# benjisu03/grayshift

Measured on AMD Instinct MI355X. Metric: Msamples/sec (primary+secondary rays), higher is better.
Workload: dtype f64; 1 GPU; C4: bouncing_spheres_50 1920x1080, 512 spp; tile=64, parallelism=tiles1, tile_plan=round-robin, collective=none, launch=one process, 1 device(s): gs_multi_create once, gs_multi_render per frame, seed=1, rays_per_frame=2921120250

## Files before the change

### __graft_entry__.py

```python
import os
import sys

ROOT = os.path.dirname(os.path.abspath(__file__))


def build():
    sys.path.insert(0, ROOT)
    from grayshift_amd import build as b
    b.build_product()
    b.build_oracle()
    b.build_kat()
    import grayshift_amd
    from grayshift_amd import _native


def smoke():
    sys.path.insert(0, ROOT)
    sys.path.insert(0, os.path.join(ROOT, "oracle"))
    import numpy as np
    import grayshift_amd as g
    from grayshift_amd import scenes
    import oracle

    sc = scenes.config("C4", width=48, spp=4)
    out, gc = g.render(sc, seed=7)
    ref, rc = oracle.render(sc, seed=7)
    d = float(np.abs(out.astype(np.float64) - ref.astype(np.float64)).max())
    if not (d < 1e-3) or gc != rc:
        raise AssertionError("smoke parity failed: max|d|=%g counters gpu=%s oracle=%s" % (d, gc, rc))
    print("smoke ok: C4 48x27x4spp max|d|=%g rays=%d" % (d, gc["rays"]))


if __name__ == "__main__":
    build()
# ... 3 lines not shown
```

### bindings/grayshift_gpu.rs

```rust
#![allow(non_camel_case_types)]

use std::os::raw::{c_char, c_void};

pub type gs_status = i32;
pub const GS_OK: gs_status = 0;
pub const GS_ERR_ARG: gs_status = -1;
pub const GS_ERR_HIP: gs_status = -2;
pub const GS_ERR_OOM: gs_status = -3;
pub const GS_ERR_UNSUPPORTED: gs_status = -4;
pub const GS_ERR_NO_DEVICE: gs_status = -5;

pub const GS_REF_SHIFT: u32 = 28;
pub const GS_REF_NONE: u32 = 0;
pub const GS_REF_NODE: u32 = 1;
pub const GS_REF_SPHERE: u32 = 2;
pub const GS_REF_MSPHERE: u32 = 3;
pub const GS_REF_QUAD: u32 = 4;
pub const GS_REF_TRIANGLE: u32 = 5;
pub const GS_REF_LIST: u32 = 6;
pub const GS_REF_INSTANCE: u32 = 7;
pub const GS_REF_MEDIUM: u32 = 8;
pub const GS_REF_BUILD_MEMBER: u32 = 15;
pub const GS_ABI_VERSION: i32 = 11;
pub const fn gs_make_ref(kind: u32, idx: u32) -> u32 { (kind << GS_REF_SHIFT) | (idx & 0x0FFF_FFFF) }
// ... 137 lines not shown
    pub feat: i32, pub node_steps: i32, pub cert_boxes: i32, pub nodes_per_leaf: f64, pub other_leaf_frac: f64,
    pub placement: i32, pub long_samples: i32, pub pilot_ms: f64,
}

#[repr(C)] #[derive(Clone, Copy)]
pub struct gs_debug_leaf_stage {
    pub tquads: *const c_void, pub n_quads: u32, pub n_cubes: u32, pub lds_quads: u32, pub lds_cubes: u32,
}

#[link(name = "grayshift")]
extern "C" {
    pub fn gs_last_error() -> *const c_char;
    pub fn gs_version() -> i32;
    pub fn gs_set_tuning(shade_batch: i32, blocks_per_cu: i32, leaf_batch: i32, sample_chunk: i32) -> gs_status;
    pub fn gs_debug_set_partial_budget(bytes: u64) -> gs_status;
    pub fn gs_debug_set_guided_tail(fine_chunk: i32, tail_pct: i32) -> gs_status;
    pub fn gs_set_node_steps(node_steps: i32) -> gs_status;
    pub fn gs_set_camera_batch(cam_batch: i32) -> gs_status;
    pub fn gs_set_placement(mode: i32) -> gs_status;
    pub fn gs_set_adaptive_mode(mode: i32) -> gs_status;
    pub fn gs_debug_set_round_items(mode: i32) -> gs_status;
    pub fn gs_debug_set_cube_lists(on: i32) -> gs_status;
    pub fn gs_debug_set_cert_boxes(on: i32) -> gs_status;
    pub fn gs_debug_set_mirror_budget(bytes: i64) -> gs_status;
    pub fn gs_debug_record_visits(scene: *const gs_device_scene, cam: *const gs_camera, ss: *const gs_sample_settings,
                                  seed: u64, part: *const gs_partition, d_packed_rgb: *mut f32, d_visits: *mut u32,
                                  stream: *mut c_void) -> gs_status;
    pub fn gs_debug_last_launch_feat(scene: *const gs_device_scene, feat: *mut i32) -> gs_status;
    pub fn gs_debug_device_scene_record(scene: *const gs_device_scene, out: *mut c_void, out_bytes: i64) -> gs_status;
    pub fn gs_debug_leaf_stage_record(scene: *const gs_device_scene, out: *mut gs_debug_leaf_stage, out_bytes: i64) -> gs_status;
    pub fn gs_device_scene_create(scene: *const gs_flat_scene, out: *mut *mut gs_device_scene) -> gs_status;
    pub fn gs_device_scene_destroy(scene: *mut gs_device_scene) -> gs_status;
    pub fn gs_device_scene_info(scene: *const gs_device_scene, out: *mut gs_scene_info) -> gs_status;
    pub fn gs_partition_capacity(cam: *const gs_camera, part: *const gs_partition) -> i64;
    pub fn gs_render_tiles_async(scene: *const gs_device_scene, cam: *const gs_camera, ss: *const gs_sample_settings,
                                 seed: u64, part: *const gs_partition, d_packed_rgb: *mut f32,
                                 d_counters: *mut gs_counters, stream: *mut c_void) -> gs_status;
    pub fn gs_render_tiles_debug_async(scene: *const gs_device_scene, cam: *const gs_camera,
                                       ss: *const gs_sample_settings, seed: u64, part: *const gs_partition,
                                       d_packed_rgb: *mut f32, d_counters: *mut gs_counters,
                                       d_item_visits: *mut u32, stream: *mut c_void) -> gs_status;
    pub fn gs_unpack_tiles_async(cam: *const gs_camera, world_size: i32, tile_w: i32, tile_h: i32, capacity: i64,
                                 d_gathered: *const f32, d_frame: *mut f32, stream: *mut c_void) -> gs_status;
    pub fn gs_render_tiles_ex_async(scene: *const gs_device_scene, cam: *const gs_camera,
                                    ss: *const gs_sample_settings, seed: u64, part: *const gs_partition,
                                    out: *const gs_render_outputs, d_counters: *mut gs_counters,
// ... 331 lines not shown
```

### grayshift_amd/_native.py

```python
import ctypes as C
import os

HERE = os.path.dirname(os.path.abspath(__file__))
LIB_PATH = os.environ.get("GS_LIB") or os.path.join(HERE, "libgrayshift.so")

GS_OBJ_SPHERE, GS_OBJ_MOVING_SPHERE, GS_OBJ_QUAD, GS_OBJ_TRIANGLE = 1, 2, 3, 4
GS_OBJ_LIST, GS_OBJ_BVH, GS_OBJ_TRANSLATE, GS_OBJ_ROTATE_Y, GS_OBJ_CUBE, GS_OBJ_MEDIUM = 5, 6, 7, 8, 9, 10
GS_MAT_LAMBERTIAN, GS_MAT_METAL, GS_MAT_DIELECTRIC, GS_MAT_DIFFUSE_LIGHT, GS_MAT_ISOTROPIC = 1, 2, 3, 4, 5
GS_TEX_SOLID, GS_TEX_CHECKERED, GS_TEX_IMAGE, GS_TEX_NOISE = 1, 2, 3, 4
GS_BG_SOLID, GS_BG_HDRI = 1, 2
GS_ABI_VERSION = 11
GS_OK, GS_ERR_ARG, GS_ERR_HIP, GS_ERR_OOM, GS_ERR_UNSUPPORTED, GS_ERR_NO_DEVICE = 0, -1, -2, -3, -4, -5

D3 = C.c_double * 3


class gs_object(C.Structure):
    _fields_ = [("kind", C.c_int32), ("material", C.c_int32), ("first", C.c_int32), ("count", C.c_int32),
                ("p", C.c_double * 9)]


class gs_material_spec(C.Structure):
    _fields_ = [("kind", C.c_int32), ("texture", C.c_int32), ("p", C.c_double * 4)]

# ... 222 lines not shown
        d["counters"] = self.counters.as_dict()
        return d


class gs_debug_leaf_stage(C.Structure):
    _fields_ = [("tquads", C.c_void_p), ("n_quads", C.c_uint32), ("n_cubes", C.c_uint32), ("lds_quads", C.c_uint32),
                ("lds_cubes", C.c_uint32)]


_P = C.c_void_p
SIGNATURES = {
    "gs_last_error": (C.c_char_p, []),
    "gs_version": (C.c_int32, []),
    "gs_set_tuning": (C.c_int32, [C.c_int32, C.c_int32, C.c_int32, C.c_int32]),
    "gs_debug_set_partial_budget": (C.c_int32, [C.c_uint64]),
    "gs_debug_set_guided_tail": (C.c_int32, [C.c_int32, C.c_int32]),
    "gs_set_node_steps": (C.c_int32, [C.c_int32]),
    "gs_set_camera_batch": (C.c_int32, [C.c_int32]),
    "gs_set_placement": (C.c_int32, [C.c_int32]),
    "gs_set_adaptive_mode": (C.c_int32, [C.c_int32]),
    "gs_debug_set_round_items": (C.c_int32, [C.c_int32]),
    "gs_debug_set_cube_lists": (C.c_int32, [C.c_int32]),
    "gs_debug_set_cert_boxes": (C.c_int32, [C.c_int32]),
    "gs_debug_set_mirror_budget": (C.c_int32, [C.c_int64]),
    "gs_debug_record_visits": (C.c_int32, [_P, C.POINTER(gs_camera), C.POINTER(gs_sample_settings), C.c_uint64,
                                           C.POINTER(gs_partition), _P, _P, _P]),
    "gs_debug_last_launch_feat": (C.c_int32, [_P, C.POINTER(C.c_int32)]),
    "gs_debug_device_scene_record": (C.c_int32, [_P, _P, C.c_int64]),
    "gs_debug_leaf_stage_record": (C.c_int32, [_P, C.POINTER(gs_debug_leaf_stage), C.c_int64]),
    "gs_device_scene_create": (C.c_int32, [_P, C.POINTER(_P)]),
    "gs_device_scene_destroy": (C.c_int32, [_P]),
    "gs_device_scene_info": (C.c_int32, [_P, C.POINTER(gs_scene_info)]),
    "gs_partition_capacity": (C.c_int64, [C.POINTER(gs_camera), C.POINTER(gs_partition)]),
    "gs_render_tiles_async": (C.c_int32, [_P, C.POINTER(gs_camera), C.POINTER(gs_sample_settings), C.c_uint64,
                                          C.POINTER(gs_partition), _P, _P, _P]),
    "gs_render_tiles_debug_async": (C.c_int32, [_P, C.POINTER(gs_camera), C.POINTER(gs_sample_settings), C.c_uint64,
                                                C.POINTER(gs_partition), _P, _P, _P, _P]),
    "gs_unpack_tiles_async": (C.c_int32, [C.POINTER(gs_camera), C.c_int32, C.c_int32, C.c_int32, C.c_int64, _P, _P,
                                          _P]),
    "gs_render_tiles_ex_async": (C.c_int32, [_P, C.POINTER(gs_camera), C.POINTER(gs_sample_settings), C.c_uint64,
                                             C.POINTER(gs_partition), C.POINTER(gs_render_outputs), _P, _P]),
    "gs_unpack_tiles_u8_async": (C.c_int32, [C.POINTER(gs_camera), C.c_int32, C.c_int32, C.c_int32, C.c_int64, _P,
                                             _P, _P]),
    "gs_ppm_max_bytes": (C.c_int64, [C.c_int32, C.c_int32]),
    "gs_ppm_scratch_bytes": (C.c_int64, [C.c_int32, C.c_int32]),
    "gs_ppm_encode_async": (C.c_int32, [_P, C.c_int32, C.c_int32, _P, C.c_int64, _P, _P, C.c_int64, _P]),
# ... 143 lines not shown
```

### grayshift_amd/build.py

```python
import argparse
import glob
import os
import subprocess
import sys

HERE = os.path.dirname(os.path.abspath(__file__))
ROOT = os.path.dirname(HERE)
LIB = os.path.join(HERE, "libgrayshift.so")
ORACLE_DIR = os.path.join(ROOT, "oracle")
ORACLE_LIB = os.path.join(ORACLE_DIR, "liboracle.so")

SOURCES = [
    os.path.join(HERE, "csrc", "device", "render.hip"),
    os.path.join(HERE, "csrc", "device", "output.hip"),
    os.path.join(HERE, "csrc", "device", "bvh_build.hip"),
    os.path.join(HERE, "csrc", "host", "scene.cpp"),
    os.path.join(HERE, "csrc", "host", "launch.cpp"),
    os.path.join(HERE, "csrc", "host", "world.cpp"),
    os.path.join(HERE, "csrc", "host", "camera.cpp"),
    os.path.join(HERE, "csrc", "host", "host_capi.cpp"),
    os.path.join(HERE, "csrc", "host", "multi_gpu.cpp"),
]


# ... 45 lines not shown
    if verbose:
        print(" ".join(cmd), flush=True)
    subprocess.run(cmd, check=True)
    os.replace(tmp, lib)
    return lib


KAT_SRC = os.path.join(ROOT, "tests", "hip", "kat_device.hip")
KAT_LIB = os.path.join(ROOT, "tests", "hip", "libkat_device.so")


def build_kat(force=False, verbose=False):
    deps = [KAT_SRC] + _headers()
    if not force and not _stale(KAT_LIB, deps):
        return KAT_LIB
    cmd = [HIPCC] + COMMON + ["-x", "hip", "--offload-arch=" + ARCH, "-shared", "-o", KAT_LIB + ".tmp", KAT_SRC]
    if verbose:
        print(" ".join(cmd), flush=True)
    subprocess.run(cmd, check=True)
    os.replace(KAT_LIB + ".tmp", KAT_LIB)
    return KAT_LIB


def build_oracle(force=False, verbose=False):
    if force and os.path.exists(ORACLE_LIB):
        os.remove(ORACLE_LIB)
    subprocess.run(["make", "-s", "-C", ORACLE_DIR], check=True,
                   stdout=None if verbose else subprocess.DEVNULL)
    return ORACLE_LIB


def main(argv=None):
    ap = argparse.ArgumentParser()
    ap.add_argument("--force", action="store_true")
    ap.add_argument("--no-oracle", action="store_true")
    ap.add_argument("-v", "--verbose", action="store_true")
    ap.add_argument("--variant", action="append", metavar="NAME:FLAGS", default=[],
                    help="also build variants/NAME.so with extra FLAGS (A/B), e.g. --variant 'v4:-DGS_MIN_WAVES=4'")
    ap.add_argument("--resource-usage", action="store_true",
                    help="print per-kernel VGPR/SGPR/LDS/occupancy (hipcc remarks)")
    a = ap.parse_args(argv)
    extra = ["-Rpass-analysis=kernel-resource-usage"] if a.resource_usage else []
    import concurrent.futures as cf

    def variant(spec):
        name, _, flags = spec.partition(":")
        path = os.path.join(HERE, "variants", name + ".so")
        os.makedirs(os.path.dirname(path), exist_ok=True)
        build_product(force=True, verbose=a.verbose, extra=extra + flags.split(), out=path)
        return "variant %s %s" % (path, flags)

    with cf.ThreadPoolExecutor(max_workers=4) as ex:
        jobs = [ex.submit(build_product, force=a.force or a.resource_usage, verbose=a.verbose, extra=extra)]
        jobs += [ex.submit(variant, spec) for spec in a.variant]
        for j in jobs[1:]:
            print(j.result())
        jobs[0].result()
    if not a.no_oracle:
        build_oracle(force=a.force, verbose=a.verbose)
        build_kat(force=a.force, verbose=a.verbose)
    print("built", LIB, "" if a.no_oracle else ORACLE_LIB)


if __name__ == "__main__":
    sys.exit(main())
```

### grayshift_amd/csrc/device/geometry.hpp

```cpp
#pragma once
#include "../../../include/grayshift_gpu.h"
#include "kernel_abi.hpp"
#include "devmath.hpp"

namespace gsd {

struct Ray {
    d3 o, d;
    double time;
};

__device__ __forceinline__ DNode load_node(const DNode* p) {
    const uint4* q = reinterpret_cast<const uint4*>(p);
    const uint4 a = q[0], b = q[1], c = q[2], d = q[3];
    DNode n;
    n.mnx = __hiloint2double((int)a.y, (int)a.x);
    n.mny = __hiloint2double((int)a.w, (int)a.z);
    n.mnz = __hiloint2double((int)b.y, (int)b.x);
    n.mxx = __hiloint2double((int)b.w, (int)b.z);
    n.mxy = __hiloint2double((int)c.y, (int)c.x);
    n.mxz = __hiloint2double((int)c.w, (int)c.z);
    n.left = d.x;
    n.right = d.y;
    n.pad0 = d.z;
// ... 109 lines not shown
    return c;
}
__device__ __forceinline__ bool box_cert_dt(float mnx, float mny, float mnz, float mxx, float mxy, float mxz,
                                            const RayCert& c, float tmin32, float closest32, float& d, float& thr) {
    const gs_f2 t0 = __builtin_elementwise_fma(gs_f2{mnx, mny}, c.ixy, c.oxy);
    const gs_f2 t1 = __builtin_elementwise_fma(gs_f2{mxx, mxy}, c.ixy, c.oxy);
    const gs_f2 tz = __builtin_elementwise_fma(gs_f2{mnz, mxz}, c.izz, c.ozz);
    const float t0x = t0.x, t1x = t1.x, t0y = t0.y, t1y = t1.y, t0z = tz.x, t1z = tz.y;
    const float lo = __builtin_fmaxf(__builtin_fmaxf(tmin32, __builtin_fminf(t0x, t1x)),
                                     __builtin_fmaxf(__builtin_fminf(t0y, t1y), __builtin_fminf(t0z, t1z)));
    const float hi = __builtin_fminf(__builtin_fminf(closest32, __builtin_fmaxf(t0x, t1x)),
                                     __builtin_fminf(__builtin_fmaxf(t0y, t1y), __builtin_fmaxf(t0z, t1z)));
    d = hi - lo;
    thr = __builtin_fmaf(GS_CERT_K, hi + lo, c.r2);
    return d > thr;
}
__device__ __forceinline__ bool box_cert(float mnx, float mny, float mnz, float mxx, float mxy, float mxz,
                                         const RayCert& c, float tmin32, float closest32, bool& undecided) {
    float d, thr;
    const bool h = box_cert_dt(mnx, mny, mnz, mxx, mxy, mxz, c, tmin32, closest32, d, thr);
    undecided = !h && d >= -thr;
    return h;
}
__device__ __forceinline__ DNode box64(const TBox& b) {
    DNode n;
    n.mnx = b.mnx;
    n.mny = b.mny;
    n.mnz = b.mnz;
    n.mxx = b.mxx;
    n.mxy = b.mxy;
    n.mxz = b.mxz;
    n.left = n.right = n.pad0 = n.pad1 = 0;
    return n;
}

__device__ __forceinline__ bool sphere_accept_rr(d3 c, double rr, const Ray& ray, double a, double tmin, double tmax,
                                            double& t_out) {
    d3 oc = sub(c, ray.o);
    double h = dot(ray.d, oc);
    double cc = len2(oc) - rr;
    double disc = h * h - a * cc;
    t_out = tmax;
    if (disc < 0.0) return false;
    double sq = sqrt(disc);
    double t = (h - sq) / a;
    if (!(tmin < t && t < tmax)) {
// ... 157 lines not shown
```

### grayshift_amd/csrc/device/kernel_abi.hpp

```cpp
#pragma once
#include <hip/hip_runtime_api.h>
#include <stddef.h>
#include <stdint.h>

#include "../../../include/grayshift_gpu.h"

#ifndef GS_BLOCK
#define GS_BLOCK 1024
#endif
#ifndef GS_MIN_WAVES
#define GS_MIN_WAVES 4
#endif
#define GS_MAX_CHAIN 16
#ifndef GS_ROUND_WHOLE_MAX_BATCH
#define GS_ROUND_WHOLE_MAX_BATCH 256
#endif
#define GS_NESTED_STACK 32
#define GS_FEAT_MEDIA 1
#define GS_FEAT_NESTED 2
#define GS_FEAT_LEAFRUN 4
#define GS_FEAT_LDSTREE 8
#define GS_FEAT_MIXED 16
#define GS_FEAT_VISITS 32
#define GS_FEAT_SPHLEAF 64
// ... 178 lines not shown
struct ViewBatch {
    gs_view v[GS_VIEW_BATCH];
    uint32_t first, n;
};
static_assert(sizeof(gs_view) % 8 == 0 && sizeof(ViewBatch) <= 3072, "gs_views_kernel copies 8-byte words of a small argument");

#define GS_ACCUM_MAX_BLOCKS 2048u
__host__ __device__ constexpr uint32_t gs_accum_blocks(uint32_t capacity) {
    return capacity == 0u ? 1u : ((capacity - 1u) / 256u + 1u < GS_ACCUM_MAX_BLOCKS ? (capacity - 1u) / 256u + 1u : GS_ACCUM_MAX_BLOCKS);
}

struct KArgs {
    const TNode* tnodes;
    const TLeaf* tleaves;
    const TBox* tboxes;
    const TQuad* tquads;
    const KParams* P;
    uint32_t root;
    int32_t shade_batch;
    int32_t leaf_batch;
    int32_t node_steps;
    int32_t cam_batch;
    int32_t cert_boxes;
    uint32_t lds_nodes;
    uint32_t lds_leaves;
    uint32_t lds_quads;
    uint32_t lds_cubes;
    const double* cubes;
    uint32_t lane_nd;
    uint32_t nest_lds;
};

#define DREF_NONE 0xFFFFFFFFu
#define DREF_LEAF (1u << GS_REF_SHIFT)
__host__ __device__ inline uint32_t device_ref(uint32_t abi_ref) {
    if (abi_ref == GS_REF_NONE) return DREF_NONE;
    if ((abi_ref >> GS_REF_SHIFT) == GS_REF_NODE) return abi_ref & GS_REF_MASK;
    return abi_ref;
}

#define THR_END 0x7FFFFFFFu
#define THR_LEAF 0x80000000u
#define THR_RET 0xFFFFFFFFu
__host__ __device__ constexpr uint32_t node_link(uint32_t pos) { return pos << 5; }

#define GS_AQ_TAG 0xFFF4A5C0u
#define GS_CUBE_FLAG 0x80000000u
#define GS_CUBE_DOUBLES 12
__host__ __device__ constexpr int cube_code(int k) { return k == 0 || k == 2 ? 4 : (k == 1 || k == 3 ? 1 : 3); }
__host__ __device__ constexpr int cube_src(int k, int f) {
    constexpr int t[6][6] = {{5, 0, 1, 6, 7, 9},    {3, 5, 1, -8, 7, -10}, {2, 3, 1, -6, 7, -9},
                             {0, 2, 1, 8, 7, 10},   {4, 0, 5, 6, -8, -11}, {1, 0, 2, 6, 8, 11}};
    return t[k][f];
}

enum { L_CSR = 0, L_CSG, L_CSB, L_LSUM, L_LSQ, L_SCOUNT, L_ND };
enum { L_ITEM = 0, L_PIX, L_BLEFT, L_SAMPLE, L_DEPTH, L_HINST, L_NI };

#ifdef GS_STAMPS
#define GS_STAMP_LDS ((GS_BLOCK / 64) * 16 * 8)
#else
#define GS_STAMP_LDS 0
#endif
enum { L_ND_CHUNKED = L_LSUM };
__host__ __device__ constexpr bool t_in_lds(int feat) {
    return (feat & (GS_FEAT_MEDIA | GS_FEAT_NESTED)) != 0 && (feat & GS_FEAT_VISITS) == 0;
// ... 22 lines not shown
```

### grayshift_amd/csrc/device/render.hip

```cpp

#include <hip/hip_runtime.h>

#include <cstdio>
#include <cmath>
#include <cstring>
#include <type_traits>

#include "../../../include/grayshift_gpu.h"
#include "kernel_abi.hpp"
#include "kernels.hpp"
#include "devmath.hpp"
#include "geometry.hpp"
#include "perlin.hpp"

using namespace gsd;

#ifndef GS_NOINLINE
#define GS_NOINLINE __forceinline__
#endif
#ifndef GS_ROUND_PIXEL_MAJOR
#define GS_ROUND_PIXEL_MAJOR 0
#endif
#ifndef GS_ROOT_RCP
#define GS_ROOT_RCP 1
#endif
#ifndef GS_PRIO_NODE
#define GS_PRIO_NODE 1
#endif
#ifndef GS_PRIO_LEAF
#define GS_PRIO_LEAF                                 \
    ((FEAT & GS_FEAT_SPHLEAF) == 0 &&                \
             ((FEAT & GS_FEAT_MIXED) == 0 || (FEAT & (GS_FEAT_MEDIA | GS_FEAT_NESTED)) != 0) \
         ? 1                                         \
         : 0)
#endif
#ifndef GS_PRIO_SHADE
#define GS_PRIO_SHADE 0
#endif
#define GS_PRIO_SET(lvl) do { if (lvl) __builtin_amdgcn_s_setprio(lvl); } while (0)
#define GS_PRIO_CLR(on) do { if (on) __builtin_amdgcn_s_setprio(0); } while (0)
#ifdef GS_ISA_MARKS
#define GS_MARK(s) asm volatile(";; GS_MARK " s)
#else
#define GS_MARK(s) do { } while (0)
#endif


enum { S_NEED = 0, S_TRACE = 1, S_SHADE = 2, S_DONE = 3, S_CAM = 4 };

#include "leaf.hpp"

__device__ __forceinline__ uint32_t node_half_b(uint32_t off) { return off + 16u; }
__device__ __forceinline__ uint32_t node_global(uint32_t off) { return off; }
template <bool LDS_ONLY>
__device__ __forceinline__ void load_tnode(const uint8_t* s_nodes, const TNode* g, uint32_t off, uint32_t lds_bytes,
                                           u32x4& a, u32x4& b) {
    if (LDS_ONLY || off < lds_bytes) {
        a = *(lds_u32x4*)(uintptr_t)off;
        b = *(lds_u32x4*)(uintptr_t)node_half_b(off);
    } else {
// ... 110 lines not shown
        for (uint32_t k = threadIdx.x; k < A.lds_cubes * (GS_CUBE_DOUBLES / 2); k += GS_BLOCK) dst[k] = src[k];
    }
    uint8_t* s_cubes = s_quads + (size_t)A.lds_quads * sizeof(TQuad);
    const QuadSrc qs{s_quads, A.tquads, A.lds_quads, s_cubes, A.lds_cubes};
    double* s_d = (double*)(s_cubes + (size_t)A.lds_cubes * (GS_CUBE_DOUBLES * 8));
    uint32_t* s_i = (uint32_t*)(s_d + A.lane_nd * GS_BLOCK);
    unsigned long long* s_cnt = (unsigned long long*)(s_i + lane_ni(FEAT) * GS_BLOCK);
#ifdef GS_STAMPS
    unsigned long long* s_reg = s_cnt + 16;
    if (threadIdx.x < (GS_BLOCK / 64) * 16) s_reg[threadIdx.x] = 0;
#endif
    if (threadIdx.x < GS_CNT_SLOTS) s_cnt[threadIdx.x] = 0;
    __syncthreads();

    const KParams* __restrict__ P = A.P;
    const DevScene& sc = P->sc;
    const gs_camera& cam = P->cam;
    const uint32_t lane = threadIdx.x & 63;
    const uint32_t tid = threadIdx.x;
    const uint64_t flushers = __builtin_amdgcn_ballot_w64(tid < GS_CNT_SLOTS);
    const double tmin = 0.001;
    constexpr int kUnroll = unroll_steps(FEAT);
    constexpr bool kSphLeaf = (FEAT & GS_FEAT_SPHLEAF) != 0;
    constexpr bool kFixed = (FEAT & GS_FEAT_FIXED) != 0;
    constexpr bool kRsplit = kFixed && (FEAT & GS_FEAT_RSPLIT) != 0;
    constexpr bool kGeneral = (FEAT & GS_FEAT_GENERAL) != 0;
    constexpr bool kViews = (FEAT & GS_FEAT_VIEWS) != 0;
#define LD(k) s_d[((k) + (t_in_lds(FEAT) ? 3 : 0)) * GS_BLOCK + tid]
#define LI(k) s_i[(k) * GS_BLOCK + tid]
    if constexpr (kSphLeaf) LI(L_HINST) = GS_REF_NONE;
    constexpr bool kNested = (FEAT & GS_FEAT_NESTED) != 0;
    uint32_t ninst_ = GS_REF_NONE;
#define LNINST (*(ninst_in_lds(FEAT) ? &s_i[lane_ninst(FEAT) * GS_BLOCK + tid] : &ninst_))
    if constexpr (kNested) LNINST = GS_REF_NONE;
    double* const s_save = s_d + (size_t)(A.lane_nd - A.nest_lds) * GS_BLOCK + tid;
    const size_t g_lanes = (size_t)gridDim.x * GS_BLOCK;
#define NSAVE(k)                                                                                   \
    (*(nest_save_lds(FEAT) && A.nest_lds ? &s_save[(size_t)(k) * GS_BLOCK]                         \
                                         : &P->nest_save[(size_t)(k) * g_lanes + (size_t)blockIdx.x * GS_BLOCK + tid]))

    uint32_t st = S_NEED;
    bool qdone = false;
    uint32_t res_base = 0, res_cnt = 0;
    uint64_t rng = 0;
    constexpr bool kTLds = t_in_lds(FEAT);
    double Tr_ = 1, Tg_ = 1, Tb_ = 1;
// ... 469 lines not shown
                                const unsigned long long k = atomicAdd(&P->counters[15], 1ull);
                                if (k < 64 && P->item_visits) {
                                    double* rec = reinterpret_cast<double*>(P->item_visits) + k * 16;
                                    const double v[16] = {ray.o.x, ray.o.y, ray.o.z, ray.d.x, ray.d.y, ray.d.z, bx.mnx,
                                                          bx.mny, bx.mnz, bx.mxx, bx.mxy, bx.mxz, tmin, closest,
                                                          (double)h, (double)closest32};
                                    for (int q = 0; q < 16; q++) rec[q] = v[q];
                                }
                            }
                        }
#endif
                    } else {
                        GS_MARK("slow_begin");
                        const bool h = box_hit(box64(A.tboxes[me >> 5]), ray.o, inv_of(ray.d), tmin, closest);
                        cur = h ? rb.z : rb.w;
                        GS_MARK("slow_end");
                    }
                }
                };
                using fast_t = std::integral_constant<bool, true>;
                using slow_t = std::integral_constant<bool, false>;
                using ldsp_t = std::integral_constant<bool, true>;
                using mixed_t = std::integral_constant<bool, false>;
                const bool lds_pass = (FEAT & GS_FEAT_LDSTREE) != 0 ||
                                      __builtin_amdgcn_ballot_w64(cur < THR_END && cur >= lim) == 0;
                if (wave_fast && lds_pass && A.node_steps >= kUnroll) {
#pragma unroll
                    for (int nstep = 0; nstep < kUnroll; nstep++) node_step(fast_t{}, ldsp_t{});
                } else if (wave_fast && lds_pass && A.node_steps == 1) {
                    node_step(fast_t{}, ldsp_t{});
                } else if (wave_fast && lds_pass) {
#pragma unroll 1
                    for (int nstep = 0; nstep < A.node_steps; nstep++) node_step(fast_t{}, ldsp_t{});
                } else if (wave_fast) {
#pragma unroll 1
                    for (int nstep = 0; nstep < A.node_steps; nstep++) node_step(fast_t{}, mixed_t{});
                } else {
#pragma unroll 1
                    for (int nstep = 0; nstep < A.node_steps; nstep++) node_step(slow_t{}, mixed_t{});
                }
                GS_MARK("node_end"); GS_PRIO_CLR(GS_PRIO_NODE);
            } else if (kNested && __builtin_amdgcn_ballot_w64(cur == THR_RET) != 0) {
#ifdef GS_STAMPS
                uint64_t rt0_;
                GS_STAMP(rt0_);
#endif
                if (cur == THR_RET) {
                    ray.o = mk(NSAVE(0), NSAVE(1), NSAVE(2));
                    ray.d = mk(NSAVE(3), NSAVE(4), NSAVE(5));
                    cur = (uint32_t)__double_as_longlong(NSAVE(6));
                    LNINST = GS_REF_NONE;
                }
                GS_REGION(6, rt0_);
            } else if (at_leaf) {
                GS_MARK("leaf_begin"); GS_PRIO_SET(GS_PRIO_LEAF);
                double scx, scy, scz, sr;
                uint32_t next, ref;
                load_tleaf<(FEAT & GS_FEAT_LDSTREE) != 0>(s_leaves, A.tleaves, cur & ~THR_LEAF, A.lds_leaves, scx, scy, scz, sr,
                                                         next, ref);
#ifndef GS_LEAF_KIND_BATCH
#define GS_LEAF_KIND_BATCH ((FEAT & (GS_FEAT_NESTED | GS_FEAT_MIXED)) != 0)
#endif
                bool take_leaf = true;
                if constexpr (GS_LEAF_KIND_BATCH && (FEAT & GS_FEAT_SPHLEAF) == 0) {
                    const uint32_t kind = ref >> GS_REF_SHIFT;
                    const uint64_t om = __builtin_amdgcn_ballot_w64(kind != GS_REF_SPHERE);
                    if (om != 0) {
                        const uint32_t k0 = __builtin_amdgcn_readlane(kind, (uint32_t)__builtin_ctzll(om));
                        take_leaf = kind == GS_REF_SPHERE || kind == k0;
                    }
                }
                if (take_leaf) {
                if constexpr ((FEAT & GS_FEAT_VISITS) != 0) {
                    if (P->visits) count_visit(P->visits, P->visit_leaf_base + (cur & ~THR_LEAF));
                }
#ifdef GS_STAMPS
                {
                    const uint64_t act = __builtin_amdgcn_read_exec();
                    const bool first = __builtin_ctzll(act) == (uint32_t)lane;
                    bool bad = false;
                    uint32_t kinds = 0;
// ... 15 lines not shown
                    const double a = len2(ray.d);
                    constexpr bool kRa = GS_ROOT_RCP && (FEAT & (GS_FEAT_MEDIA | GS_FEAT_NESTED)) == 0;
                    if (kRa && __builtin_amdgcn_ballot_w64(!(a >= 0x1p-900 && a <= 0x1p900)) == 0)
                        return sphere_accept_rr_ra(c, rr, ray, a, rcp_cert(a), tmin, closest, t);
                    return sphere_accept_rr(c, rr, ray, a, tmin, closest, t);
                };
                auto sphere_leaf = [&]() __attribute__((always_inline)) {
                    GS_MARK("sphere_begin");
                    count_sph();
                    double t;
                    if (sphere_test(mk(scx, scy, scz), sr, t)) {
                        closest = t;
                        closest32 = (float)t;
                        hit_ref = ref;
                        if constexpr (kNested) LI(L_HINST) = LNINST;
                        else if constexpr (!kSphLeaf) LI(L_HINST) = GS_REF_NONE;
                    }
                    GS_MARK("sphere_end");
                };
                if constexpr ((FEAT & GS_FEAT_SPHLEAF) != 0) {
                    const bool two = cur_next_is_leaf(next);
                    double s2x, s2y, s2z, s2r;
                    uint32_t next2, ref2;
                    load_tleaf<(FEAT & GS_FEAT_LDSTREE) != 0>(s_leaves, A.tleaves, two ? next & ~THR_LEAF : cur & ~THR_LEAF,
                                                             A.lds_leaves, s2x, s2y, s2z, s2r, next2, ref2);
                    const double a = len2(ray.d);
                    const SphereDisc q1 = sphere_disc_rr(mk(scx, scy, scz), sr, ray, a);
                    const SphereDisc q2 = sphere_disc_rr(mk(s2x, s2y, s2z), s2r, ray, a);
                    const bool real1 = !(q1.disc < 0.0), real2 = two && !(q2.disc < 0.0);
                    GS_MARK("sphere_begin");
                    double t;
                    const double ra = rcp_cert(a);
                    const bool wave_ra =
                        GS_ROOT_RCP && __builtin_amdgcn_ballot_w64(!(a >= 0x1p-900 && a <= 0x1p900)) == 0;
                    auto take = [&](double hh, double dd) __attribute__((always_inline)) {
                        return wave_ra ? sphere_root_take_ra(hh, dd, a, ra, tmin, closest, t)
                                       : sphere_root_take(hh, dd, a, tmin, closest, t);
                    };
                    if (real1 || real2) {
                        const double hA = real1 ? q1.h : q2.h, dA = real1 ? q1.disc : q2.disc;
                        if (take(hA, dA)) {
                            closest = t;
                            hit_ref = real1 ? ref : ref2;
                        }
                    }
                    if (real1 && real2) {
                        if (take(q2.h, q2.disc)) {
// ... 1024 lines not shown
```

### grayshift_amd/csrc/host/launch.cpp

```cpp
#include <algorithm>
#include <chrono>
#include <cmath>
#include <cstring>

#include "../device/kernels.hpp"
#include "render_host.hpp"

static thread_local std::string tl_err;
static std::atomic<int32_t> g_shade_batch{0};
static std::atomic<int32_t> g_blocks_per_cu{0};
static std::atomic<int32_t> g_node_steps{0};
static std::atomic<int32_t> g_leaf_batch{0};
static std::atomic<int32_t> g_cam_batch{0};
static std::atomic<int32_t> g_tail_pct{0};
static std::atomic<int32_t> g_sample_chunk{-1};
static std::atomic<int32_t> g_placement{1};
static std::atomic<uint64_t> g_partial_budget{4ull << 30};
static std::atomic<int32_t> g_adaptive_rounds{1};
static std::atomic<int32_t> g_round_whole{0};
#ifndef GS_ROUND_MIN_CAP
#define GS_ROUND_MIN_CAP 512
#endif
static const uint64_t kMaxRounds = 1u << 16;
static std::atomic<int32_t> g_cube_lists{1};
static std::atomic<int32_t> g_cert_boxes{1};
static std::atomic<int64_t> g_mirror_budget{-1};

Knobs read_knobs() {
    const auto rlx = std::memory_order_relaxed;
    Knobs k;
    k.shade_batch = g_shade_batch.load(rlx);
    k.blocks_per_cu = g_blocks_per_cu.load(rlx);
    k.node_steps = g_node_steps.load(rlx);
    k.leaf_batch = g_leaf_batch.load(rlx);
    k.cam_batch = g_cam_batch.load(rlx);
    k.tail_pct = g_tail_pct.load(rlx);
    k.sample_chunk = g_sample_chunk.load(rlx);
    k.placement = g_placement.load(rlx);
    k.partial_budget = g_partial_budget.load(rlx);
    k.adaptive_rounds = g_adaptive_rounds.load(rlx);
    k.round_whole = g_round_whole.load(rlx);
    k.cube_lists = g_cube_lists.load(rlx);
    k.cert_boxes = g_cert_boxes.load(rlx);
    k.mirror_budget = g_mirror_budget.load(rlx);
    return k;
}

int32_t launch_node_steps(const gs_device_scene* ds, const Knobs& k) {
    return std::max(1, std::min<int32_t>(unroll_steps(ds->feat), k.node_steps > 0 ? k.node_steps : ds->node_steps));
}

extern "C" void gs_set_last_error(const char* msg) { tl_err = msg ? msg : ""; }
gs_status fail(gs_status code, const std::string& msg) {
    tl_err = msg;
    return code;
}

extern "C" {

const char* gs_last_error(void) { return tl_err.c_str(); }
int32_t gs_version(void) { return GS_ABI_VERSION; }

gs_status gs_set_node_steps(int32_t node_steps) {
    if (node_steps < 0 || node_steps > GS_NODE_STEPS) return fail(GS_ERR_ARG, "node_steps outside [0, GS_NODE_STEPS]");
    g_node_steps = node_steps;
    return GS_OK;
// ... 24 lines not shown

gs_status gs_set_adaptive_mode(int32_t mode) {
    if (mode < 0 || mode > 2)
        return fail(GS_ERR_ARG, "adaptive mode is 0 (per-lane loop), 1 (auto) or 2 (batch rounds)");
    g_adaptive_rounds = mode;
    return GS_OK;
}

gs_status gs_debug_set_round_items(int32_t mode) {
    if (mode < -1 || mode > 1) return fail(GS_ERR_ARG, "round item mode is -1 (auto), 0 (split) or 1 (whole)");
    g_round_whole = mode;
    return GS_OK;
}

gs_status gs_debug_set_cube_lists(int32_t on) {
    if (on != 0 && on != 1) return fail(GS_ERR_ARG, "cube lists are 0 (the list loop) or 1 (cube_test)");
    g_cube_lists = on;
    return GS_OK;
}

gs_status gs_debug_set_cert_boxes(int32_t on) {
    if (on != 0 && on != 1) return fail(GS_ERR_ARG, "cert boxes are 1 (the 1e15 rule decides) or 0 (the f64 box test)");
    g_cert_boxes = on;
    return GS_OK;
}

gs_status gs_debug_set_mirror_budget(int64_t bytes) {
    if (bytes < -1) return fail(GS_ERR_ARG, "the mirror budget is -1 (the block's own) or a byte count >= 0");
    g_mirror_budget = bytes;
    return GS_OK;
}

gs_status gs_debug_set_partial_budget(uint64_t bytes) {
    g_partial_budget.store(bytes ? bytes : (4ull << 30));
    return GS_OK;
}

gs_status gs_debug_set_guided_tail(int32_t fine_chunk, int32_t tail_pct) {
    if (fine_chunk < 0 || tail_pct < 0) return fail(GS_ERR_ARG, "fine_chunk and tail_pct are >= 0 (0: the default)");
    if (fine_chunk > 1) return fail(GS_ERR_ARG, "fine_chunk is 0 or 1 (1-sample tail items)");
    g_tail_pct.store(tail_pct);
    return GS_OK;
}

#ifndef GS_SHORT_SAMPLE_LANE_US
#define GS_SHORT_SAMPLE_LANE_US 50.0
// ... 576 lines not shown
    kp.direct = q.direct ? 1u : 0u;
    kp.zero_counters = q.zero_counters && q.d_counters ? 1u : 0u;
    kp.counters = (unsigned long long*)q.d_counters;
    kp.item_visits = q.outs->item_visits;
    kp.visits = q.va ? q.va->visits : nullptr;
    kp.visit_leaf_base = q.va ? q.va->leaf_base : 0u;
    const uint64_t waves = (uint64_t)blocks * (GS_BLOCK / 64);
    kp.waves = (uint32_t)waves;
    kp.lanes = (uint32_t)(blocks * GS_BLOCK);
    const uint64_t claim_cap = kp.chunk && kp.chunk <= 4u ? (uint64_t)GS_CLAIM_FINE : 32u;
    kp.claim = (uint32_t)std::max<uint64_t>(1, std::min<uint64_t>(claim_cap, (uint64_t)kp.n_items / waves / GS_CLAIM_DIV));
    kp.claim_fine = (uint32_t)std::max<uint64_t>(1, std::min<uint64_t>(GS_CLAIM_FINE, (uint64_t)kp.n_items / waves / GS_CLAIM_DIV));
    return kp;
}

static KArgs fill_args(const gs_device_scene* ds, const gs_device_scene::LaunchCfg& lc, bool chunked, const Knobs& k) {
    KArgs a{};
    a.tnodes = ds->dev.tnodes;
    a.tboxes = ds->dev.tboxes;
    a.tleaves = ds->dev.tleaves;
    a.tquads = ds->tquads;
    a.root = ds->thr_root;
    a.cert_boxes = ds->cert_boxes ? 1 : 0;
    a.shade_batch = k.shade_batch > 0 ? k.shade_batch : ds->shade_batch;
    a.leaf_batch = std::max<int32_t>(1, k.leaf_batch > 0 ? k.leaf_batch : ds->leaf_batch);
    a.node_steps = launch_node_steps(ds, k);
    a.cam_batch = std::max<int32_t>(1, k.cam_batch > 0 ? k.cam_batch : ds->cam_batch);
    a.lds_nodes = lc.mirror.nodes;
    a.lds_leaves = lc.mirror.leaves;
    a.lds_quads = lc.mirror.quads;
    a.lds_cubes = lc.mirror.cubes;
    a.cubes = ds->dev.cubes;
    a.lane_nd = lane_nd(chunked, ds->feat) + lc.nest_lds;
    a.nest_lds = lc.nest_lds;
    return a;
}

static int pick_slot(gs_device_scene* ds, hipStream_t st, size_t need_partial) {
    for (int k = 0; k < kLaunchSlots; k++)
        if (ds->slots[k].used && ds->slots[k].stream == st) return k;
    int idle = -1;
    for (int k = 0; k < kLaunchSlots; k++) {
        LaunchSlot& c = ds->slots[k];
        if (c.used && hipEventQuery(c.done) != hipSuccess) continue;
        if (c.partial_bytes >= need_partial) return k;
        if (idle < 0) idle = k;
// ... 536 lines not shown
```

### grayshift_amd/csrc/host/render_host.hpp

```cpp
#pragma once
#include <atomic>
#include <mutex>
#include <string>
#include <vector>

#include "../device/kernel_abi.hpp"
#include "internal.hpp"

gs_status fail(gs_status code, const std::string& msg);
#define HIPCHK(x)                                                                               \
    do {                                                                                        \
        hipError_t e_ = (x);                                                                    \
        if (e_ != hipSuccess) return fail(GS_ERR_HIP, std::string(#x) + ": " + hipGetErrorString(e_)); \
    } while (0)

struct Knobs {
    int32_t shade_batch;
    int32_t blocks_per_cu;
    int32_t node_steps;
    int32_t leaf_batch;
    int32_t cam_batch;
    int32_t tail_pct;
    int32_t sample_chunk;
    int32_t placement;
    uint64_t partial_budget;
    int32_t adaptive_rounds;
    int32_t round_whole;
    int32_t cube_lists;
    int32_t cert_boxes;
    int64_t mirror_budget;
};
Knobs read_knobs();

struct MirrorPrefix {
    uint32_t nodes = 0, leaves = 0, quads = 0, cubes = 0;
    int64_t bytes() const {
        return (int64_t)nodes * (int64_t)sizeof(TNode) + (int64_t)leaves * (int64_t)sizeof(TLeaf) +
               (int64_t)quads * (int64_t)sizeof(TQuad) + (int64_t)cubes * (GS_CUBE_DOUBLES * 8);
    }
};

struct LaunchSlot {
    KParams* params = nullptr;
    uint32_t* queue = nullptr;
    double* partial = nullptr;
    size_t partial_bytes = 0;
    hipEvent_t done = nullptr;
    hipStream_t stream = nullptr;
    bool used = false;
    void* rbuf = nullptr;
    size_t rbuf_bytes = 0;
    double* nest_save = nullptr;
// ... 77 lines not shown
```

### include/grayshift_gpu.h

```cpp
#ifndef GRAYSHIFT_GPU_H
#define GRAYSHIFT_GPU_H

#include <stddef.h>
#include <stdint.h>
#include "grayshift_scene.h"

#ifdef __cplusplus
extern "C" {
#endif

#define GS_ABI_VERSION 11

typedef int32_t gs_status;
enum {
    GS_OK = 0,
    GS_ERR_ARG = -1,
    GS_ERR_HIP = -2,
    GS_ERR_OOM = -3,
    GS_ERR_UNSUPPORTED = -4,
    GS_ERR_NO_DEVICE = -5
};

#define GS_REF_SHIFT 28u
#define GS_REF_MASK 0x0FFFFFFFu
// ... 139 lines not shown

const char* gs_last_error(void);
int32_t gs_version(void);

gs_status gs_set_tuning(int32_t shade_batch, int32_t blocks_per_cu, int32_t leaf_batch, int32_t sample_chunk);

gs_status gs_set_node_steps(int32_t node_steps);

gs_status gs_set_camera_batch(int32_t cam_batch);

gs_status gs_set_placement(int32_t mode);

gs_status gs_debug_record_visits(const gs_device_scene* scene, const gs_camera* cam,
                                 const gs_sample_settings* ss, uint64_t seed, const gs_partition* part,
                                 float* d_packed_rgb, uint32_t* d_visits, void* stream);

gs_status gs_set_adaptive_mode(int32_t mode);

gs_status gs_debug_set_round_items(int32_t mode);

gs_status gs_debug_set_cube_lists(int32_t on);

gs_status gs_debug_set_cert_boxes(int32_t on);

gs_status gs_debug_set_mirror_budget(int64_t bytes);

gs_status gs_debug_set_partial_budget(uint64_t bytes);

gs_status gs_debug_set_guided_tail(int32_t fine_chunk, int32_t tail_pct);

gs_status gs_debug_last_launch_feat(const gs_device_scene* scene, int32_t* feat);

gs_status gs_debug_device_scene_record(const gs_device_scene* scene, void* out, int64_t out_bytes);

typedef struct gs_debug_leaf_stage {
    const void* tquads;
    uint32_t n_quads, n_cubes;
    uint32_t lds_quads, lds_cubes;
} gs_debug_leaf_stage;
gs_status gs_debug_leaf_stage_record(const gs_device_scene* scene, gs_debug_leaf_stage* out, int64_t out_bytes);

gs_status gs_device_scene_create(const gs_flat_scene* scene, gs_device_scene** out);
gs_status gs_device_scene_destroy(gs_device_scene* scene);

typedef struct gs_scene_info {
    uint32_t node_records, leaf_records;
// ... 253 lines not shown
```

Before: 8932 Msamples/s.

## Add certified f32 sphere-miss prefilter to skip f64 leaf tests

```diff
diff --git a/__graft_entry__.py b/__graft_entry__.py
--- a/__graft_entry__.py
+++ b/__graft_entry__.py
@@ -10,6 +10,7 @@
     b.build_product()
     b.build_oracle()
     b.build_kat()
+    b.build_scert()
     import grayshift_amd
     from grayshift_amd import _native
 
diff --git a/bindings/grayshift_gpu.rs b/bindings/grayshift_gpu.rs
--- a/bindings/grayshift_gpu.rs
+++ b/bindings/grayshift_gpu.rs
@@ -183,6 +183,7 @@
     pub fn gs_debug_set_round_items(mode: i32) -> gs_status;
     pub fn gs_debug_set_cube_lists(on: i32) -> gs_status;
     pub fn gs_debug_set_cert_boxes(on: i32) -> gs_status;
+    pub fn gs_debug_set_cert_spheres(on: i32) -> gs_status;
     pub fn gs_debug_set_mirror_budget(bytes: i64) -> gs_status;
     pub fn gs_debug_record_visits(scene: *const gs_device_scene, cam: *const gs_camera, ss: *const gs_sample_settings,
                                   seed: u64, part: *const gs_partition, d_packed_rgb: *mut f32, d_visits: *mut u32,
diff --git a/grayshift_amd/_native.py b/grayshift_amd/_native.py
--- a/grayshift_amd/_native.py
+++ b/grayshift_amd/_native.py
@@ -268,6 +268,7 @@
     "gs_debug_set_round_items": (C.c_int32, [C.c_int32]),
     "gs_debug_set_cube_lists": (C.c_int32, [C.c_int32]),
     "gs_debug_set_cert_boxes": (C.c_int32, [C.c_int32]),
+    "gs_debug_set_cert_spheres": (C.c_int32, [C.c_int32]),
     "gs_debug_set_mirror_budget": (C.c_int32, [C.c_int64]),
     "gs_debug_record_visits": (C.c_int32, [_P, C.POINTER(gs_camera), C.POINTER(gs_sample_settings), C.c_uint64,
                                            C.POINTER(gs_partition), _P, _P, _P]),
diff --git a/grayshift_amd/build.py b/grayshift_amd/build.py
--- a/grayshift_amd/build.py
+++ b/grayshift_amd/build.py
@@ -91,6 +91,22 @@
     return KAT_LIB
 
 
+SCERT_SRC = os.path.join(ROOT, "tests", "hip", "sphere_cert_host.hip")
+SCERT_LIB = os.path.join(ROOT, "tests", "hip", "libsphere_cert_host.so")
+
+
+def build_scert(force=False, verbose=False):
+    deps = [SCERT_SRC] + _headers()
+    if not force and not _stale(SCERT_LIB, deps):
+        return SCERT_LIB
+    cmd = [HIPCC] + COMMON + ["-x", "hip", "--cuda-host-only", "-shared", "-o", SCERT_LIB + ".tmp", SCERT_SRC]
+    if verbose:
+        print(" ".join(cmd), flush=True)
+    subprocess.run(cmd, check=True)
+    os.replace(SCERT_LIB + ".tmp", SCERT_LIB)
+    return SCERT_LIB
+
+
 def build_oracle(force=False, verbose=False):
     if force and os.path.exists(ORACLE_LIB):
         os.remove(ORACLE_LIB)
@@ -128,6 +144,7 @@
     if not a.no_oracle:
         build_oracle(force=a.force, verbose=a.verbose)
         build_kat(force=a.force, verbose=a.verbose)
+        build_scert(force=a.force, verbose=a.verbose)
     print("built", LIB, "" if a.no_oracle else ORACLE_LIB)
 
 
diff --git a/grayshift_amd/csrc/device/geometry.hpp b/grayshift_amd/csrc/device/geometry.hpp
--- a/grayshift_amd/csrc/device/geometry.hpp
+++ b/grayshift_amd/csrc/device/geometry.hpp
@@ -155,6 +155,28 @@
     undecided = !h && d >= -thr;
     return h;
 }
+#define GS_SCERT_K 3.814697265625e-06f
+__host__ __device__ __forceinline__ bool sphere_cert_miss_f32(float ox, float oy, float oz, float dx, float dy, float dz,
+                                                              float cx, float cy, float cz, float rr) {
+    const float ex = cx - ox, ey = cy - oy, ez = cz - oz;
+    const float wx = __builtin_fmaf(ey, dz, -(ez * dy));
+    const float wy = __builtin_fmaf(ez, dx, -(ex * dz));
+    const float wz = __builtin_fmaf(ex, dy, -(ey * dx));
+    const float W2 = __builtin_fmaf(wx, wx, __builtin_fmaf(wy, wy, wz * wz));
+    const float a2 = __builtin_fmaf(dx, dx, __builtin_fmaf(dy, dy, dz * dz));
+    const float S = __builtin_fmaxf(__builtin_fabsf(cx), __builtin_fmaxf(__builtin_fabsf(cy), __builtin_fabsf(cz))) +
+                    __builtin_fmaxf(__builtin_fabsf(ox), __builtin_fmaxf(__builtin_fabsf(oy), __builtin_fabsf(oz)));
+    const float m2 = __builtin_fmaf(S, S, rr);
+    const float rhs = __builtin_fmaf(a2, __builtin_fmaf(GS_SCERT_K, m2, rr), 1e-30f);
+    const bool in_range = a2 >= 1e-12f && a2 <= 1e12f && m2 >= 1e-12f && m2 <= 1e24f;
+    return in_range && W2 > rhs;
+}
+__host__ __device__ __forceinline__ bool sphere_cert_miss(const d3& o, const d3& d, double cx, double cy, double cz,
+                                                          double rr) {
+    return sphere_cert_miss_f32((float)o.x, (float)o.y, (float)o.z, (float)d.x, (float)d.y, (float)d.z, (float)cx,
+                                (float)cy, (float)cz, (float)rr);
+}
+
 __device__ __forceinline__ DNode box64(const TBox& b) {
     DNode n;
     n.mnx = b.mnx;
diff --git a/grayshift_amd/csrc/device/kernel_abi.hpp b/grayshift_amd/csrc/device/kernel_abi.hpp
--- a/grayshift_amd/csrc/device/kernel_abi.hpp
+++ b/grayshift_amd/csrc/device/kernel_abi.hpp
@@ -224,6 +224,7 @@
     int32_t node_steps;
     int32_t cam_batch;
     int32_t cert_boxes;
+    int32_t cert_spheres;
     uint32_t lds_nodes;
     uint32_t lds_leaves;
     uint32_t lds_quads;
@@ -244,6 +245,7 @@
 #define THR_END 0x7FFFFFFFu
 #define THR_LEAF 0x80000000u
 #define THR_RET 0xFFFFFFFFu
+#define THR_UNDEC 0x40000000u
 __host__ __device__ constexpr uint32_t node_link(uint32_t pos) { return pos << 5; }
 
 #define GS_AQ_TAG 0xFFF4A5C0u
diff --git a/grayshift_amd/csrc/device/render.hip b/grayshift_amd/csrc/device/render.hip
--- a/grayshift_amd/csrc/device/render.hip
+++ b/grayshift_amd/csrc/device/render.hip
@@ -36,6 +36,9 @@
 #endif
 #ifndef GS_PRIO_SHADE
 #define GS_PRIO_SHADE 0
+#endif
+#ifndef GS_LEAF_RUN
+#define GS_LEAF_RUN 2
 #endif
 #define GS_PRIO_SET(lvl) do { if (lvl) __builtin_amdgcn_s_setprio(lvl); } while (0)
 #define GS_PRIO_CLR(on) do { if (on) __builtin_amdgcn_s_setprio(0); } while (0)
@@ -192,6 +195,8 @@
     const double tmin = 0.001;
     constexpr int kUnroll = unroll_steps(FEAT);
     constexpr bool kSphLeaf = (FEAT & GS_FEAT_SPHLEAF) != 0;
+    constexpr bool kSphCert = kSphLeaf && (FEAT & GS_FEAT_VISITS) == 0;
+    constexpr uint32_t kLeafIdx = kSphCert ? ~(THR_LEAF | THR_UNDEC) : ~THR_LEAF;
     constexpr bool kFixed = (FEAT & GS_FEAT_FIXED) != 0;
     constexpr bool kRsplit = kFixed && (FEAT & GS_FEAT_RSPLIT) != 0;
     constexpr bool kGeneral = (FEAT & GS_FEAT_GENERAL) != 0;
@@ -707,6 +712,36 @@
                 using slow_t = std::integral_constant<bool, false>;
                 using ldsp_t = std::integral_constant<bool, true>;
                 using mixed_t = std::integral_constant<bool, false>;
+#ifndef GS_SCERT_PLACE
+#define GS_SCERT_PLACE 1
+#endif
+                auto sphere_filter = [&]() __attribute__((always_inline)) {
+                    if constexpr (kSphCert) {
+                        if (A.cert_spheres == 0) return;
+                        const bool cand = cur > THR_END && (cur & THR_UNDEC) == 0;
+                        if (__builtin_amdgcn_ballot_w64(cand) == 0) return;
+                        GS_MARK("scert_begin");
+                        if (cand) {
+                            if (!fast) cur |= THR_UNDEC;
+#pragma unroll 1
+                            for (int k = 0; k < GS_LEAF_RUN && cur > THR_END && (cur & THR_UNDEC) == 0; k++) {
+                                double fx, fy, fz, frr;
+                                uint32_t fnext, fref;
+                                load_tleaf<(FEAT & GS_FEAT_LDSTREE) != 0>(s_leaves, A.tleaves, cur & ~THR_LEAF, A.lds_leaves,
+                                                                         fx, fy, fz, frr, fnext, fref);
+                                const bool miss = sphere_cert_miss(ray.o, ray.d, fx, fy, fz, frr);
+#ifdef GS_CERT_CHECK
+                                if (miss && !(sphere_disc_rr(mk(fx, fy, fz), frr, ray, len2(ray.d)).disc < 0.0))
+                                    atomicAdd(&P->counters[15], 1ull);
+#endif
+                                c_sph += miss ? 1u : 0u;
+                                cur = miss ? fnext : cur | THR_UNDEC;
+                            }
+                        }
+                        GS_MARK("scert_end");
+                    }
+                };
+                if constexpr ((GS_SCERT_PLACE & 2) != 0) sphere_filter();
                 const bool lds_pass = (FEAT & GS_FEAT_LDSTREE) != 0 ||
                                       __builtin_amdgcn_ballot_w64(cur < THR_END && cur >= lim) == 0;
                 if (wave_fast && lds_pass && A.node_steps >= kUnroll) {
@@ -724,6 +759,7 @@
 #pragma unroll 1
                     for (int nstep = 0; nstep < A.node_steps; nstep++) node_step(slow_t{}, mixed_t{});
                 }
+                if constexpr ((GS_SCERT_PLACE & 1) != 0) sphere_filter();
                 GS_MARK("node_end"); GS_PRIO_CLR(GS_PRIO_NODE);
             } else if (kNested && __builtin_amdgcn_ballot_w64(cur == THR_RET) != 0) {
 #ifdef GS_STAMPS
@@ -741,7 +777,7 @@
                 GS_MARK("leaf_begin"); GS_PRIO_SET(GS_PRIO_LEAF);
                 double scx, scy, scz, sr;
                 uint32_t next, ref;
-                load_tleaf<(FEAT & GS_FEAT_LDSTREE) != 0>(s_leaves, A.tleaves, cur & ~THR_LEAF, A.lds_leaves, scx, scy, scz, sr,
+                load_tleaf<(FEAT & GS_FEAT_LDSTREE) != 0>(s_leaves, A.tleaves, cur & kLeafIdx, A.lds_leaves, scx, scy, scz, sr,
                                                          next, ref);
 #ifndef GS_LEAF_KIND_BATCH
 #define GS_LEAF_KIND_BATCH ((FEAT & (GS_FEAT_NESTED | GS_FEAT_MIXED)) != 0)
@@ -803,7 +839,7 @@
                     const bool two = cur_next_is_leaf(next);
                     double s2x, s2y, s2z, s2r;
                     uint32_t next2, ref2;
-                    load_tleaf<(FEAT & GS_FEAT_LDSTREE) != 0>(s_leaves, A.tleaves, two ? next & ~THR_LEAF : cur & ~THR_LEAF,
+                    load_tleaf<(FEAT & GS_FEAT_LDSTREE) != 0>(s_leaves, A.tleaves, two ? next & ~THR_LEAF : cur & kLeafIdx,
                                                              A.lds_leaves, s2x, s2y, s2z, s2r, next2, ref2);
                     const double a = len2(ray.d);
                     const SphereDisc q1 = sphere_disc_rr(mk(scx, scy, scz), sr, ray, a);
diff --git a/grayshift_amd/csrc/host/launch.cpp b/grayshift_amd/csrc/host/launch.cpp
--- a/grayshift_amd/csrc/host/launch.cpp
+++ b/grayshift_amd/csrc/host/launch.cpp
@@ -24,6 +24,7 @@
 static const uint64_t kMaxRounds = 1u << 16;
 static std::atomic<int32_t> g_cube_lists{1};
 static std::atomic<int32_t> g_cert_boxes{1};
+static std::atomic<int32_t> g_cert_spheres{1};
 static std::atomic<int64_t> g_mirror_budget{-1};
 
 Knobs read_knobs() {
@@ -42,6 +43,7 @@
     k.round_whole = g_round_whole.load(rlx);
     k.cube_lists = g_cube_lists.load(rlx);
     k.cert_boxes = g_cert_boxes.load(rlx);
+    k.cert_spheres = g_cert_spheres.load(rlx);
     k.mirror_budget = g_mirror_budget.load(rlx);
     return k;
 }
@@ -112,6 +114,12 @@
 gs_status gs_debug_set_cert_boxes(int32_t on) {
     if (on != 0 && on != 1) return fail(GS_ERR_ARG, "cert boxes are 1 (the 1e15 rule decides) or 0 (the f64 box test)");
     g_cert_boxes = on;
+    return GS_OK;
+}
+
+gs_status gs_debug_set_cert_spheres(int32_t on) {
+    if (on != 0 && on != 1) return fail(GS_ERR_ARG, "cert spheres are 1 (the certified f32 sphere miss filters leaf lanes) or 0 (every sphere takes the f64 test)");
+    g_cert_spheres = on;
     return GS_OK;
 }
 
@@ -734,6 +742,7 @@
     a.tquads = ds->tquads;
     a.root = ds->thr_root;
     a.cert_boxes = ds->cert_boxes ? 1 : 0;
+    a.cert_spheres = k.cert_spheres ? 1 : 0;
     a.shade_batch = k.shade_batch > 0 ? k.shade_batch : ds->shade_batch;
     a.leaf_batch = std::max<int32_t>(1, k.leaf_batch > 0 ? k.leaf_batch : ds->leaf_batch);
     a.node_steps = launch_node_steps(ds, k);
diff --git a/grayshift_amd/csrc/host/render_host.hpp b/grayshift_amd/csrc/host/render_host.hpp
--- a/grayshift_amd/csrc/host/render_host.hpp
+++ b/grayshift_amd/csrc/host/render_host.hpp
@@ -28,6 +28,7 @@
     int32_t round_whole;
     int32_t cube_lists;
     int32_t cert_boxes;
+    int32_t cert_spheres;
     int64_t mirror_budget;
 };
 Knobs read_knobs();
diff --git a/include/grayshift_gpu.h b/include/grayshift_gpu.h
--- a/include/grayshift_gpu.h
+++ b/include/grayshift_gpu.h
@@ -185,6 +185,8 @@
 gs_status gs_debug_set_cube_lists(int32_t on);
 
 gs_status gs_debug_set_cert_boxes(int32_t on);
+
+gs_status gs_debug_set_cert_spheres(int32_t on);
 
 gs_status gs_debug_set_mirror_budget(int64_t bytes);
 
```

Result: slower. 7784 Msamples/s (-12.9%).
